# Arcadia-Science/arcadia-microscopy-tools

Measured on AMD Instinct MI355X. Metric: fields-of-view/sec (4x2048^2 uint16) end-to-end segment+props, higher is better.
Workload: dtype f64; 1 GPU; configs[2]: synthetic 4-channel 2048x2048 uint16 FOVs, DAPI Gaussian+Otsu+open/close+EDT+peak markers+watershed nuclei (SEEDED relief, seeds_first: marker pixels spread first in raster order, cannot tie; SURVEY A.8's plain -EDT relief with exact ties is reported under sublines.a8_exact) + clear_border/relabel + morphology and 4-channel intensity regionprops; mode=weak scaling, 192 FOVs per GPU per step, streams_per_gpu=4, fovs_per_launch=48, max_cells_per_fov=2048, distinct_fovs_per_gpu=8, resident_in_hbm=True

## Files before the change

### arcadia_microscopy_tools_amd/csrc/amt_edt.hip

```cpp
#include "amt_internal.h"

constexpr unsigned G_INF = 0xFFFFu;

__global__ void __launch_bounds__(256) edt_zero_words_kernel(const uint8_t* __restrict__ mask, unsigned long long* __restrict__ zw,
                                                             int H, int W, int WW, size_t nwords, int fast) {
    const size_t i = (size_t)blockIdx.x * 256 + threadIdx.x;
    if (i >= nwords) return;
    const int wi = (int)(i % WW);
    const size_t row = i / WW;
    const uint8_t* p = mask + row * W + (size_t)wi * 64;
    const int valid = W - wi * 64 < 64 ? W - wi * 64 : 64;
    unsigned long long z = 0;
    if (fast) {
        uint4 q[4];
#pragma unroll
        for (int j = 0; j < 4; ++j) q[j] = *reinterpret_cast<const uint4*>(p + (16 * j < valid ? 16 * j : 0));
#pragma unroll
        for (int j = 0; j < 4; ++j) {
            const unsigned v[4] = {q[j].x, q[j].y, q[j].z, q[j].w};
            unsigned sixteen = 0;
#pragma unroll
            for (int k = 0; k < 4; ++k) {
                const unsigned nz = ((((v[k] & 0x7F7F7F7Fu) + 0x7F7F7F7Fu) | v[k]) >> 7) & 0x01010101u;
                sixteen |= (((nz ^ 0x01010101u) * 0x01020408u) >> 24) << (4 * k);
            }
            if (16 * j < valid) z |= (unsigned long long)(sixteen & 0xFFFFu) << (16 * j);
        }
    } else {
        for (int k = 0; k < valid; ++k) z |= (unsigned long long)(p[k] == 0) << k;
    }
    zw[i] = z;
}

__device__ __forceinline__ unsigned edt_g_at(const unsigned long long* __restrict__ zr, int WW, int x) {
    const int wi = x >> 6, bit = x & 63;
    const unsigned long long own = zr[wi];
    if ((own >> bit) & 1ull) return 0u;
    unsigned dl = G_INF, dr = G_INF;
    unsigned long long m = own & ((1ull << bit) - 1ull);
    int w = wi;
    while (m == 0 && w > 0) m = zr[--w];
    if (m) dl = (unsigned)(x - (w * 64 + 63 - __clzll((long long)m)));
    m = bit == 63 ? 0ull : (own >> (bit + 1)) << (bit + 1);
    w = wi;
    while (m == 0 && w + 1 < WW) m = zr[++w];
    if (m) dr = (unsigned)(w * 64 + __ffsll((long long)m) - 1 - x);
    const unsigned d = dl < dr ? dl : dr;
    return d >= G_INF ? G_INF : d;
}

template <int EC_ROWS, int EC_HALO>
__global__ void __launch_bounds__(256) edt_bits_kernel(const unsigned long long* __restrict__ zw, int* __restrict__ d2_out,
                                                       double* __restrict__ edt_out, int H, int W, int WW) {
    constexpr int EC_TROWS = EC_ROWS + 2 * EC_HALO;
    __shared__ __attribute__((aligned(16))) unsigned short tile[EC_TROWS][64];
    __shared__ unsigned long long zs[EC_TROWS][3];
    const int lane = threadIdx.x & 63, wave = threadIdx.x >> 6;
    const int wi = blockIdx.x;
    const int y0 = blockIdx.y * EC_ROWS;
    const size_t plane = (size_t)blockIdx.z * H * W;
    const unsigned long long* zp = zw + (size_t)blockIdx.z * H * WW;
    for (int i = threadIdx.x; i < EC_TROWS * 3; i += 256) {
        const int r = i / 3, c = i - r * 3;
        const int y = y0 - EC_HALO + r, w = wi - 1 + c;
        zs[r][c] = (y >= 0 && y < H && w >= 0 && w < WW) ? zp[(size_t)y * WW + w] : 0ull;
    }
    __syncthreads();
    constexpr unsigned BIG = 0x20000u;
    for (int task = threadIdx.x; task < EC_TROWS * 8; task += 256) {
        const int r = task >> 3, b = task & 7;
        const int y = y0 - EC_HALO + r;
        uint4 out = make_uint4(0xFFFFFFFFu, 0xFFFFFFFFu, 0xFFFFFFFFu, 0xFFFFFFFFu);
        if (y >= 0 && y < H) {
            const int bit0 = b * 8, x0 = wi * 64 + bit0;
            const unsigned long long own = zs[r][1];
            const unsigned z8 = (unsigned)(own >> bit0) & 0xffu;
            out = make_uint4(0u, 0u, 0u, 0u);
            if (z8 != 0xffu) {
                unsigned dl = BIG, dr = BIG;
                unsigned long long m = own & ((1ull << bit0) - 1ull);
                int w = wi;
                if (m == 0 && w > 0) {
                    m = zs[r][0];
                    --w;
                    const unsigned long long* zr = zp + (size_t)y * WW;
                    while (m == 0 && w > 0) m = zr[--w];
                }
                if (m) dl = (unsigned)(x0 - (w * 64 + 63 - __clzll((long long)m)));
                const int sh = bit0 + 8;
                m = sh == 64 ? 0ull : (own >> sh) << sh;
                w = wi;
                if (m == 0 && w + 1 < WW) {
                    m = zs[r][2];
                    ++w;
                    const unsigned long long* zr = zp + (size_t)y * WW;
                    while (m == 0 && w + 1 < WW) m = zr[++w];
                }
                if (m) dr = (unsigned)(w * 64 + __ffsll((long long)m) - 1 - (x0 + 7));
                unsigned L[8], R[8];
#pragma unroll
                for (int i = 0; i < 8; ++i) {
                    const unsigned prev = i == 0 ? dl : L[i - 1] + 1u;
                    L[i] = ((z8 >> i) & 1u) ? 0u : (prev < BIG ? prev : BIG);
                }
#pragma unroll
                for (int i = 7; i >= 0; --i) {
                    const unsigned nxt = i == 7 ? dr : R[i + 1] + 1u;
                    R[i] = ((z8 >> i) & 1u) ? 0u : (nxt < BIG ? nxt : BIG);
                }
                unsigned d[8];
#pragma unroll
                for (int i = 0; i < 8; ++i) {
                    const unsigned mn = L[i] < R[i] ? L[i] : R[i];
                    d[i] = mn >= G_INF ? G_INF : mn;
                }
                out.x = d[0] | (d[1] << 16);
                out.y = d[2] | (d[3] << 16);
                out.z = d[4] | (d[5] << 16);
                out.w = d[6] | (d[7] << 16);
            }
        }
        *reinterpret_cast<uint4*>(&tile[r][b * 8]) = out;
    }
    __syncthreads();
    const int c4 = (lane & 15) * 4, rsub = lane >> 4;
    const int xg = wi * 64 + c4;
    if (xg >= W) return;
    const bool vec = xg + 3 < W && (W & 3) == 0 && (!d2_out || (reinterpret_cast<uintptr_t>(d2_out) & 15) == 0) &&
                     (!edt_out || (reinterpret_cast<uintptr_t>(edt_out) & 15) == 0);
#pragma unroll 1
    for (int j = 0; j < EC_ROWS / 16; ++j) {
        const int ly = EC_HALO + wave * (EC_ROWS / 4) + rsub + 4 * j;
        const int y = y0 - EC_HALO + ly;
        if (y >= H) continue;
        unsigned best[4];
        {
            const uint2 gq = *reinterpret_cast<const uint2*>(&tile[ly][c4]);
            const unsigned g0[4] = {gq.x & 0xFFFFu, gq.x >> 16, gq.y & 0xFFFFu, gq.y >> 16};
#pragma unroll
            for (int i = 0; i < 4; ++i) best[i] = g0[i] == G_INF ? 0xFFFFFFFFu : g0[i] * g0[i];
        }
        for (unsigned k = 1; k <= (unsigned)EC_HALO; ++k) {
            const unsigned kk = k * k;
            if (!(kk < best[0] || kk < best[1] || kk < best[2] || kk < best[3])) break;
            const uint2 uq = *reinterpret_cast<const uint2*>(&tile[ly - (int)k][c4]);
            const uint2 dq = *reinterpret_cast<const uint2*>(&tile[ly + (int)k][c4]);
            const unsigned gu[4] = {uq.x & 0xFFFFu, uq.x >> 16, uq.y & 0xFFFFu, uq.y >> 16};
            const unsigned gd[4] = {dq.x & 0xFFFFu, dq.x >> 16, dq.y & 0xFFFFu, dq.y >> 16};
#pragma unroll
            for (int i = 0; i < 4; ++i) {
                const unsigned gm = gu[i] < gd[i] ? gu[i] : gd[i];
                const unsigned c = gm == G_INF ? 0xFFFFFFFFu : kk + gm * gm;
                best[i] = c < best[i] ? c : best[i];
            }
        }
#pragma unroll
        for (int i = 0; i < 4; ++i) {
            unsigned bq = best[i];
            const int x = xg + i;
            if (bq != 0 && x < W) {
                for (unsigned kk = EC_HALO + 1; kk < 65536u && (unsigned long long)kk * kk < bq; ++kk) {
                    const int yu = y - (int)kk, yd = y + (int)kk;
                    if (yu < 0 && yd >= H) break;
                    unsigned gm = G_INF;
                    if (yu >= 0) gm = edt_g_at(zp + (size_t)yu * WW, WW, x);
                    if (yd < H) {
                        const unsigned gd = edt_g_at(zp + (size_t)yd * WW, WW, x);
                        gm = gd < gm ? gd : gm;
                    }
                    if (gm != G_INF) {
                        const unsigned c = kk * kk + gm * gm;
                        bq = c < bq ? c : bq;
                    }
                }
                if (bq > 0x7fffffffu) bq = (unsigned)(y + 1) * (unsigned)(y + 1) + (unsigned)x * (unsigned)x;
            }
            best[i] = bq;
        }
        const size_t i0 = plane + (size_t)y * W + xg;
        if (vec) {
            if (d2_out) *reinterpret_cast<int4*>(d2_out + i0) = make_int4((int)best[0], (int)best[1], (int)best[2], (int)best[3]);
            if (edt_out) {
                *reinterpret_cast<double2*>(edt_out + i0) = make_double2(sqrt((double)best[0]), sqrt((double)best[1]));
                *reinterpret_cast<double2*>(edt_out + i0 + 2) = make_double2(sqrt((double)best[2]), sqrt((double)best[3]));
            }
        } else {
            for (int i = 0; i < 4 && xg + i < W; ++i) {
                if (d2_out) d2_out[i0 + i] = (int)best[i];
                if (edt_out) edt_out[i0 + i] = sqrt((double)best[i]);
            }
        }
    }
}

extern "C" int amt_edt(amt_ctx* ctx, const uint8_t* mask, int32_t* d2_out, double* edt_out, int nplanes, int H,
                       int W) {
    AMT_CHECK_OPERANDS("amt_edt", amt_in("mask", mask, amt_span(1, nplanes, H, W)), amt_out("d2_out", d2_out, amt_span(4, nplanes, H, W)),
                       amt_out("edt_out", edt_out, amt_span(8, nplanes, H, W)));
    AMT_TRY(amt_set_device(ctx));
    AMT_REQUIRE(mask && (d2_out || edt_out) && nplanes >= 0 && H > 0 && W > 0, "edt: bad arguments");
    AMT_REQUIRE(H <= 32768 && W <= 32768, "edt: image larger than 32768 pixels per side");
    if (nplanes == 0) return AMT_OK;
    const size_t tiles64 = (size_t)((W + 63) / 64) * ((H + 63) / 64) * nplanes;
    const int WW = (W + 63) / 64;
    const size_t nwords = (size_t)nplanes * H * WW;
    amt_scratch s(ctx);
    amt_buf<unsigned long long> zw(s, nwords);
    AMT_TRY(s.commit());
    const int fast = W % 16 == 0 && (reinterpret_cast<uintptr_t>(mask) & 15) == 0;
    hipLaunchKernelGGL(edt_zero_words_kernel, dim3((unsigned)((nwords + 255) / 256)), dim3(256), 0, ctx->stream, mask, zw, H,
                       W, WW, nwords, fast);
    AMT_LAUNCH_CHECK();
    if (tiles64 >= 4096 && !edt_out)
        hipLaunchKernelGGL((edt_bits_kernel<64, 16>), dim3(WW, (H + 63) / 64, nplanes), dim3(256), 0, ctx->stream, zw, d2_out,
                           edt_out, H, W, WW);
    else
        hipLaunchKernelGGL((edt_bits_kernel<32, 24>), dim3(WW, (H + 31) / 32, nplanes), dim3(256), 0, ctx->stream, zw, d2_out,
                           edt_out, H, W, WW);
    AMT_LAUNCH_CHECK();
    return AMT_OK;
}

constexpr int PK_MAXM = 16;
constexpr int PKR_ROWS = 64, PKR_IN = 62, PKR_BATCH = 22, PKR_NBATCH = (PKR_ROWS + 2) / PKR_BATCH;
static_assert(PKR_BATCH * PKR_NBATCH == PKR_ROWS + 2, "row batches must tile the strip");
constexpr int PKM_CNT_STRIDE = 32;

template <bool LIST>
__global__ void __launch_bounds__(256) peaks_rows_kernel(const int* __restrict__ d2, const uint8_t* __restrict__ mask,
                                                         uint8_t* __restrict__ peaks, int H, int W, int m,
                                                         int* __restrict__ found, int* __restrict__ fcount, int cap) {
    const int lane = threadIdx.x & 63;
    const int strip = blockIdx.x * 4 + (threadIdx.x >> 6);
    if (strip * PKR_IN >= W) return;
    const size_t base = (size_t)blockIdx.z * H * W;
    const int* D = d2 + base;
    const int x = strip * PKR_IN - 1 + lane;
    const int y0 = blockIdx.y * PKR_ROWS;
    const bool xin = x >= 0 && x < W;
    const bool xok = xin && lane >= 1 && lane <= PKR_IN && x >= m && x < W - m;
    const int side = 2 * m + 1, wsize = side * side;

    const int xc = x < 0 ? 0 : (x < W ? x : W - 1);
    auto load_row = [&](int y) -> int {
        const int yc = y < 0 ? 0 : (y < H ? y : H - 1);
        return D[(size_t)yc * W + xc];
    };
    int npk = 0, mypk = 0;
    auto flush = [&]() {
        int at = 0;
        if (lane == 0) at = atomicAdd(&fcount[(size_t)blockIdx.z * PKM_CNT_STRIDE], npk);
        at = __shfl(at, 0) + lane;
        if (lane < npk && at < cap) found[(size_t)blockIdx.z * cap + at] = mypk;
        npk = 0;
    };
    int cur[PKR_BATCH], nxt[PKR_BATCH];
#pragma unroll
    for (int j = 0; j < PKR_BATCH; ++j) cur[j] = load_row(y0 - 1 + j);
    int v1 = 0, v1l = 0, v1r = 0, h1 = 0, h2 = 0;
    for (int b = 0; b < PKR_NBATCH; ++b) {
        if (b + 1 < PKR_NBATCH) {
#pragma unroll
            for (int j = 0; j < PKR_BATCH; ++j) nxt[j] = load_row(y0 - 1 + (b + 1) * PKR_BATCH + j);
        }
#pragma unroll
        for (int j = 0; j < PKR_BATCH; ++j) {
            const int r = y0 - 1 + b * PKR_BATCH + j;
            const int v0 = (xin && r >= 0 && r < H) ? cur[j] : 0;
            if (__ballot(v0 > 0 || v1 > 0) == 0ull) {
                h2 = h1, h1 = 0, v1 = 0, v1l = 0, v1r = 0;
                continue;
            }
            const int v0l = amt_lane_left(v0), v0r = amt_lane_right(v0);
            int h0 = v0 > v0l ? v0 : v0l;
            h0 = h0 > v0r ? h0 : v0r;
            const int yc = r - 1;
            bool cand = xok && v1 > 0 && yc >= y0 && yc < y0 + PKR_ROWS && yc >= m && yc < H - m;
            if (m >= 1) {
                int nb = h0 > h2 ? h0 : h2;
                nb = nb > v1l ? nb : v1l;
                nb = nb > v1r ? nb : v1r;
                cand = cand && !(nb > v1);
            }
            unsigned long long todo = __ballot(cand);
            while (todo) {
                const int sl = __ffsll((long long)todo) - 1;
                todo &= todo - 1ull;
                const int sv = __shfl(v1, sl);
                const int sx = strip * PKR_IN - 1 + sl;
                bool gt = false;
                for (int k = lane; k < wsize; k += 64) {
                    const int dy = k / side, dx = k - dy * side;
                    gt |= D[(size_t)(yc - m + dy) * W + (sx - m + dx)] > sv;
                }
                const bool hit = __ballot(gt) == 0ull && lane == sl && mask[base + (size_t)yc * W + sx];
                if (hit) peaks[base + (size_t)yc * W + sx] = 1;
                if (LIST && __ballot(hit) != 0ull) {
                    if (lane == npk) mypk = yc * W + sx;
                    if (++npk == 64) flush();
                }
            }
            h2 = h1, h1 = h0;
            v1 = v0, v1l = v0l, v1r = v0r;
        }
#pragma unroll
        for (int j = 0; j < PKR_BATCH; ++j) cur[j] = nxt[j];
    }
    if (LIST && npk) flush();
}

__global__ void __launch_bounds__(256) peaks_unwrite_kernel(const int* __restrict__ list, const int* __restrict__ count,
                                                            const int* __restrict__ status, uint8_t* __restrict__ peaks,
                                                            size_t n, int cap) {
    uint8_t* o = peaks + (size_t)blockIdx.y * n;
    if (status[blockIdx.y] < 0) {
        for (size_t i = (size_t)blockIdx.x * 256 + threadIdx.x; i < n; i += (size_t)gridDim.x * 256) o[i] = 0;
        return;
    }
    const int K = count[blockIdx.y] < cap ? count[blockIdx.y] : cap;
    const int* lst = list + (size_t)blockIdx.y * cap;
    for (int k = blockIdx.x * 256 + threadIdx.x; k < K; k += gridDim.x * 256) o[lst[k]] = 0;
}

extern "C" int amt_peak_mask(amt_ctx* ctx, const int32_t* d2, const uint8_t* mask, uint8_t* peaks, int nplanes, int H,
                             int W, int min_distance, const int32_t* prev_list, const int32_t* prev_count, int capacity,
                             const int32_t* prev_status) {
    AMT_REQUIRE(!prev_list == !prev_count && !prev_list == !prev_status,
                "peak_mask: the previous run's peak lists, counts and label counts go together");
    AMT_REQUIRE(!prev_list || capacity >= 1, "peak_mask: the previous run's list capacity must be positive");
    AMT_CHECK_OPERANDS("amt_peak_mask", amt_in("d2", d2, amt_span(4, nplanes, H, W)), amt_in("mask", mask, amt_span(1, nplanes, H, W)),
                       amt_out("peaks", peaks, amt_span(1, nplanes, H, W)),
                       amt_in("prev_list", prev_list, amt_span(4, nplanes, capacity)),
                       amt_in("prev_count", prev_count, amt_span(4, nplanes)),
                       amt_in("prev_status", prev_status, amt_span(4, nplanes)));
    AMT_TRY(amt_set_device(ctx));
    AMT_REQUIRE(d2 && mask && peaks && nplanes >= 0 && H > 0 && W > 0, "peak_mask: bad arguments");
    AMT_REQUIRE(min_distance >= 0 && min_distance <= PK_MAXM, "peak_mask: min_distance %d out of range 0..%d",
                min_distance, PK_MAXM);
    if (nplanes == 0) return AMT_OK;
    const int m = min_distance;
    if (prev_list) {
        hipLaunchKernelGGL(peaks_unwrite_kernel, dim3(amt_grid_for((size_t)capacity, 256, 64), nplanes), dim3(256), 0,
                           ctx->stream, prev_list, prev_count, prev_status, peaks, (size_t)H * W, capacity);
        AMT_LAUNCH_CHECK();
    } else {
        AMT_HIP_CHECK(hipMemsetAsync(peaks, 0, (size_t)nplanes * H * W, ctx->stream));
    }
    const int nstrips = (W + PKR_IN - 1) / PKR_IN;
    dim3 grid((nstrips + 3) / 4, (H + PKR_ROWS - 1) / PKR_ROWS, nplanes);
    hipLaunchKernelGGL(peaks_rows_kernel<false>, grid, dim3(256), 0, ctx->stream, d2, mask, peaks, H, W, m, (int*)nullptr,
                       (int*)nullptr, 0);
    AMT_LAUNCH_CHECK();
    return AMT_OK;
}

constexpr int PKM_TIER = AMT_PEAK_MARKERS_LDS_TIER;
constexpr int PKM_THREADS = 1024;
static_assert(2 * PKM_TIER * sizeof(int) <= 36 * 1024 - 256, "list + parents of the LDS tier stay below 36 KB");

__global__ void __launch_bounds__(256) peaks_clear_kernel(const int* __restrict__ list, const int* __restrict__ count,
                                                          const int* __restrict__ status, uint8_t* __restrict__ peaks,
                                                          int* __restrict__ markers, int* __restrict__ fcount, size_t n,
                                                          int cap) {
    if (blockIdx.x == 0 && threadIdx.x == 0) fcount[(size_t)blockIdx.y * PKM_CNT_STRIDE] = 0;
    uint8_t* pk = peaks + (size_t)blockIdx.y * n;
    int* mk = markers + (size_t)blockIdx.y * n;
    if (status[blockIdx.y] < 0) {
        for (size_t i = (size_t)blockIdx.x * 256 + threadIdx.x; i < n; i += (size_t)gridDim.x * 256) pk[i] = 0, mk[i] = 0;
        return;
    }
    const int K = count[blockIdx.y] < cap ? count[blockIdx.y] : cap;
    const int* lst = list + (size_t)blockIdx.y * cap;
    for (int k = blockIdx.x * 256 + threadIdx.x; k < K; k += gridDim.x * 256) {
        const int p = lst[k];
        pk[p] = 0;
        mk[p] = 0;
    }
}

__device__ __forceinline__ void pkm_exchange(int* a, int i, int l, int n) {
    if (l < n) {
        const int u = a[i], v = a[l];
        if (u > v) a[i] = v, a[l] = u;
    }
}
__device__ __forceinline__ void pkm_sort(int* a, int n) {
    int n2 = 1;
    while (n2 < n) n2 <<= 1;
    const int pairs = n2 >> 1;
    for (int k = 2; k <= n2; k <<= 1) {
        const int hk = k >> 1;
        for (int t = threadIdx.x; t < pairs; t += PKM_THREADS) {
            const int i = ((t & ~(hk - 1)) << 1) | (t & (hk - 1));
            pkm_exchange(a, i, i ^ (k - 1), n);
        }
        __syncthreads();
        for (int j = hk >> 1; j > 0; j >>= 1) {
            for (int t = threadIdx.x; t < pairs; t += PKM_THREADS) {
                const int i = ((t & ~(j - 1)) << 1) | (t & (j - 1));
                pkm_exchange(a, i, i | j, n);
            }
            __syncthreads();
        }
    }
}

template <bool LDS>
__device__ __forceinline__ int pkm_label(int* lst, int* par, int K, int W, int conn8, int* __restrict__ mk,
                                         int* __restrict__ kl, int* wsum) {
    const int tid = threadIdx.x;
    pkm_sort(lst, K);
    for (int k = tid; k < K; k += PKM_THREADS) {
        par[k] = k;
        if (kl) kl[k] = lst[k];
    }
    __syncthreads();
    for (int k = tid; k < K; k += PKM_THREADS) {
        const int p = lst[k];
        const int y = p / W, x = p - y * W;
        if (x > 0 && k > 0 && lst[k - 1] == p - 1) {
            if (LDS) lds_union(par, k, k - 1); else uf_union(par, k, k - 1);
        }
        if (y == 0) continue;
        const int north = p - W;
        int lo = 0, hi = k;
        while (lo < hi) {
            const int mid = (lo + hi) >> 1;
            if (lst[mid] < north) lo = mid + 1; else hi = mid;
        }
        const bool up = lst[lo] == north;
        if (up) {
            if (LDS) lds_union(par, k, lo); else uf_union(par, k, lo);
        }
        if (conn8) {
// ... 20 lines not shown
    int rank = incl - mine, total = 0;
    for (int w = 0; w < PKM_THREADS / 64; ++w) {
        if (w < wave) rank += wsum[w];
        total += wsum[w];
    }
    for (int k = b; k < e; ++k)
        if (par[k] == k) par[k] = ~(rank++);
    __syncthreads();
    for (int k = tid; k < K; k += PKM_THREADS) {
        int v = par[k];
        if (v >= 0) v = par[v];
        mk[lst[k]] = -v;
    }
    return total;
}

__global__ void __launch_bounds__(PKM_THREADS) sp_markers_kernel(int* found, const int* __restrict__ fcount, int* gpar,
                                                                 int* __restrict__ markers, int* __restrict__ count_dev,
                                                                 int* __restrict__ keep_list, int* __restrict__ keep_count,
                                                                 size_t n, int W, int cap, int conn8) {
    __shared__ int s_lst[PKM_TIER], s_par[PKM_TIER];
    __shared__ int s_wsum[PKM_THREADS / 64];
    const int plane = blockIdx.x;
    const int K = fcount[(size_t)plane * PKM_CNT_STRIDE];
    if (K > cap) {
        if (threadIdx.x == 0) {
            count_dev[plane] = -1;
            if (keep_count) keep_count[plane] = 0;
        }
        return;
    }
    int* fl = found + (size_t)plane * cap;
    int* mk = markers + (size_t)plane * n;
    int* kl = keep_list ? keep_list + (size_t)plane * cap : nullptr;
    int nroots;
    if (K <= PKM_TIER) {
        for (int k = threadIdx.x; k < K; k += PKM_THREADS) s_lst[k] = fl[k];
        __syncthreads();
        nroots = pkm_label<true>(s_lst, s_par, K, W, conn8, mk, kl, s_wsum);
    } else {
        nroots = pkm_label<false>(fl, gpar + (size_t)plane * cap, K, W, conn8, mk, kl, s_wsum);
    }
    if (threadIdx.x == 0) {
        count_dev[plane] = nroots;
        if (keep_count) keep_count[plane] = K;
    }
}

extern "C" int amt_peak_markers(amt_ctx* ctx, const int32_t* d2, const uint8_t* mask, uint8_t* peaks, int32_t* markers,
                                int32_t* count_dev, int nplanes, int H, int W, int min_distance, int connectivity,
                                int capacity, int32_t* keep_list, int32_t* keep_count) {
    AMT_REQUIRE(!keep_list == !keep_count, "peak_markers: keep_list and keep_count go together");
    AMT_CHECK_OPERANDS("amt_peak_markers", amt_in("d2", d2, amt_span(4, nplanes, H, W)), amt_in("mask", mask, amt_span(1, nplanes, H, W)),
                       amt_out("peaks", peaks, amt_span(1, nplanes, H, W)), amt_out("markers", markers, amt_span(4, nplanes, H, W)),
                       amt_out("count_dev", count_dev, amt_span(4, nplanes)),
                       amt_out("keep_list", keep_list, amt_span(4, nplanes, capacity)),
                       amt_out("keep_count", keep_count, amt_span(4, nplanes)));
    AMT_REQUIRE(d2 && mask && peaks && markers && count_dev && nplanes >= 0 && H > 0 && W > 0,
                "peak_markers: bad arguments");
    AMT_REQUIRE(min_distance >= 0 && min_distance <= PK_MAXM, "peak_markers: min_distance %d out of range 0..%d",
                min_distance, PK_MAXM);
    AMT_REQUIRE(connectivity == 1 || connectivity == 2, "peak_markers: connectivity must be 1 or 2");
    AMT_REQUIRE(capacity >= 1, "peak_markers: capacity must be positive");
    AMT_REQUIRE((size_t)H * W < 0x7fffffffull, "peak_markers: plane too large");
    AMT_TRY(amt_set_device(ctx));
    if (nplanes == 0) return AMT_OK;
    const size_t n = (size_t)H * W;
    const size_t capn = (size_t)nplanes * capacity;
    amt_scratch s(ctx);
    amt_buf<int> found(s, capn);
    amt_buf<int> parent(s, capn);
    amt_buf<int> fcount(s, (size_t)nplanes * PKM_CNT_STRIDE);
    AMT_TRY(s.commit());
    if (keep_list) {
        hipLaunchKernelGGL(peaks_clear_kernel, dim3(amt_grid_for((size_t)capacity, 256, 64), nplanes), dim3(256), 0,
                           ctx->stream, (const int*)keep_list, (const int*)keep_count, (const int*)count_dev, peaks, markers,
                           (int*)fcount, n, capacity);
        AMT_LAUNCH_CHECK();
    } else {
        AMT_HIP_CHECK(hipMemsetAsync(peaks, 0, (size_t)nplanes * n, ctx->stream));
        AMT_HIP_CHECK(hipMemsetAsync(markers, 0, (size_t)nplanes * n * sizeof(int32_t), ctx->stream));
        AMT_HIP_CHECK(hipMemsetAsync(fcount, 0, (size_t)nplanes * PKM_CNT_STRIDE * sizeof(int), ctx->stream));
    }
    const int nstrips = (W + PKR_IN - 1) / PKR_IN;
    dim3 grid((nstrips + 3) / 4, (H + PKR_ROWS - 1) / PKR_ROWS, nplanes);
    hipLaunchKernelGGL(peaks_rows_kernel<true>, grid, dim3(256), 0, ctx->stream, d2, mask, peaks, H, W, min_distance,
                       (int*)found, (int*)fcount, capacity);
    AMT_LAUNCH_CHECK();
    hipLaunchKernelGGL(sp_markers_kernel, dim3(nplanes), dim3(PKM_THREADS), 0, ctx->stream, (int*)found,
                       (const int*)fcount, (int*)parent, markers, count_dev, keep_list, keep_count, n, W, capacity,
                       connectivity == 2 ? 1 : 0);
    AMT_LAUNCH_CHECK();
    return AMT_OK;
}
```

### arcadia_microscopy_tools_amd/csrc/amt_props.hip

```cpp
#include "amt_internal.h"
#include "amt_perlabel.h"

#include <vector>

typedef unsigned long long u64;

enum { A_N = 0, A_SY, A_SX, A_SYY, A_SXX, A_SXY, A_C1, A_C2, A_C3, A_NACC };

__global__ void __launch_bounds__(256) rp_init_kernel(u64* __restrict__ acc, int* __restrict__ bbox, size_t nlab) {
    for (size_t i = (size_t)blockIdx.x * 256 + threadIdx.x; i < nlab; i += (size_t)gridDim.x * 256) {
        if (acc)
            for (int k = 0; k < A_NACC; ++k) acc[i * A_NACC + k] = 0;
        bbox[i * 4 + 0] = 0x7fffffff;
        bbox[i * 4 + 1] = 0x7fffffff;
        bbox[i * 4 + 2] = -1;
        bbox[i * 4 + 3] = -1;
    }
}

__device__ __forceinline__ double diff_of_products(u64 a, u64 b, u64 c, u64 d) {
    u64 lo1 = a * b, hi1 = __umul64hi(a, b);
    u64 lo2 = c * d, hi2 = __umul64hi(c, d);
    bool neg = (hi1 < hi2) || (hi1 == hi2 && lo1 < lo2);
    u64 hi, lo;
// ... 469 lines not shown
    const int2* r = rows + (size_t)plane * cap + off;
    int2* CL = chainL + (size_t)plane * 3 * cap + 3 * off;
    int2* CR = chainR + (size_t)plane * 3 * cap + 3 * off;
    int nl = 0, nr = 0;
    for (int Y = 2 * miny - 1; Y <= 2 * maxy + 1; ++Y) {
        int mn = 0x7fffffff, mx = -0x7fffffff;
        if (Y & 1) {
            int ya = (Y - 1) / 2, yb = (Y + 1) / 2;
            if (Y < 0) {
                ya = -1;
                yb = 0;
            }
            if (ya >= miny && ya <= maxy) {
                int2 e = r[ya - miny];
                if (e.y >= e.x) {
                    mn = min(mn, 2 * e.x);
                    mx = max(mx, 2 * e.y);
                }
            }
            if (yb >= miny && yb <= maxy) {
                int2 e = r[yb - miny];
                if (e.y >= e.x) {
                    mn = min(mn, 2 * e.x);
                    mx = max(mx, 2 * e.y);
                }
            }
        } else {
            int2 e = r[Y / 2 - miny];
            if (e.y >= e.x) {
                mn = 2 * e.x - 1;
                mx = 2 * e.y + 1;
            }
        }
        if (mx < mn) continue;
        while (nl >= 2) {
            int2 p0 = CL[nl - 2], p1 = CL[nl - 1];
            long long cr = (long long)(p1.x - p0.x) * (mn - p0.y) - (long long)(p1.y - p0.y) * (Y - p0.x);
            if (cr <= 0) --nl; else break;
        }
        CL[nl++] = make_int2(Y, mn);
        while (nr >= 2) {
            int2 p0 = CR[nr - 2], p1 = CR[nr - 1];
            long long cr = (long long)(p1.x - p0.x) * (mx - p0.y) - (long long)(p1.y - p0.y) * (Y - p0.x);
            if (cr >= 0) --nr; else break;
        }
        CR[nr++] = make_int2(Y, mx);
    }
    long long count = 0;
    int il = 0, ir = 0;
    for (int y = miny; y <= maxy; ++y) {
        const int Y = 2 * y;
        while (il + 1 < nl && CL[il + 1].x <= Y) ++il;
        while (ir + 1 < nr && CR[ir + 1].x <= Y) ++ir;
        long long xmin, xmax;
        {
            int2 p0 = CL[il];
            if (p0.x == Y || il + 1 >= nl) {
                xmin = ceil_div(p0.y, 2);
            } else {
                int2 p1 = CL[il + 1];
                long long dY = p1.x - p0.x;
                long long num = (long long)p0.y * dY + (long long)(p1.y - p0.y) * (Y - p0.x);
                xmin = ceil_div(num, 2 * dY);
            }
        }
        {
            int2 p0 = CR[ir];
            if (p0.x == Y || ir + 1 >= nr) {
                xmax = floor_div(p0.y, 2);
            } else {
                int2 p1 = CR[ir + 1];
                long long dY = p1.x - p0.x;
                long long num = (long long)p0.y * dY + (long long)(p1.y - p0.y) * (Y - p0.x);
                xmax = floor_div(num, 2 * dY);
            }
        }
        if (CROWS) crows[(size_t)plane * cap + off + (y - miny)] = make_int2((int)xmin, (int)xmax);
        else if (xmax >= xmin) count += xmax - xmin + 1;
    }
    if (!CROWS) rp_write_convex(trow, (double)count);
}

constexpr int HULL_CH = 2 * HULL_HMAX + 1;
__device__ __forceinline__ int floor_div32(int a, int b) {
    const int q = a / b;
    return (a % b != 0 && a < 0) ? q - 1 : q;
}
__device__ __forceinline__ int ceil_div32(int a, int b) {
    const int q = a / b;
    return (a % b != 0 && a > 0) ? q + 1 : q;
}
template <bool CROWS>
__global__ void __launch_bounds__(64) rp_hull_lds_kernel(const int* __restrict__ bbox, const int* __restrict__ hoff,
                                                         const int* __restrict__ htot, const int2* __restrict__ rows,
                                                         size_t cap, double* __restrict__ table, int max_label,
                                                         int2* __restrict__ crows) {
    __shared__ unsigned short s_rows[HULL_HMAX * 32];
    __shared__ unsigned short s_ch[HULL_CH * 64];
    const int plane = blockIdx.y;
    const int lane = threadIdx.x, side = lane & 1, pr = lane >> 1;
    const int l = blockIdx.x * 32 + pr;
    if (l >= max_label) return;
    const size_t li = (size_t)plane * max_label + l;
    double* trow = CROWS ? nullptr : table + li * AMT_RP_NCOLS;
    const int miny = bbox[li * 4 + 0], x0 = bbox[li * 4 + 1], maxy = bbox[li * 4 + 2], x1 = bbox[li * 4 + 3];
    if (maxy < miny) {
        if (!CROWS && side == 0) trow[AMT_RP_AREA_CONVEX] = 0.0;
        return;
    }
    const int h = maxy - miny + 1;
    if (h > HULL_HMAX || x1 - x0 + 1 > HULL_WMAX) return;
    const size_t off = (size_t)hoff[li];
    if ((size_t)htot[plane] > cap || off + (size_t)h > cap) {
        if (!CROWS && side == 0) rp_write_convex(trow, __longlong_as_double(0x7ff8000000000000ll));
        return;
    }
    const int2* r = rows + (size_t)plane * cap + off;
    for (int k0 = side; k0 < h; k0 += 16) {
        int2 e[8];
#pragma unroll
        for (int u = 0; u < 8; ++u) e[u] = r[min(k0 + 2 * u, h - 1)];
#pragma unroll
        for (int u = 0; u < 8; ++u)
            if (k0 + 2 * u < h)
                s_rows[(k0 + 2 * u) * 32 + pr] =
                    e[u].y >= e[u].x ? (unsigned short)((e[u].x - x0) | ((e[u].y - x0) << 8)) : (unsigned short)255;
    }
    __builtin_amdgcn_s_waitcnt(0);
    __builtin_amdgcn_wave_barrier();
    int nc = 0;
    for (int Yr = 0; Yr <= 2 * h; ++Yr) {
        int mn = 0x7fffffff, mx = -1;
        if (!(Yr & 1)) {
            const int ka = (Yr >> 1) - 1, kb = Yr >> 1;
            if (ka >= 0) {
                const unsigned e = s_rows[ka * 32 + pr];
                if ((e >> 8) >= (e & 255)) {
                    mn = min(mn, 2 * (int)(e & 255) + 1);
                    mx = max(mx, 2 * (int)(e >> 8) + 1);
                }
            }
            if (kb < h) {
                const unsigned e = s_rows[kb * 32 + pr];
                if ((e >> 8) >= (e & 255)) {
                    mn = min(mn, 2 * (int)(e & 255) + 1);
                    mx = max(mx, 2 * (int)(e >> 8) + 1);
                }
            }
        } else {
            const unsigned e = s_rows[(Yr >> 1) * 32 + pr];
            if ((e >> 8) >= (e & 255)) {
                mn = 2 * (int)(e & 255);
                mx = 2 * (int)(e >> 8) + 2;
            }
        }
        if (mx < mn) continue;
        const int val = side ? mx : mn;
        while (nc >= 2) {
            const int v0 = s_ch[(nc - 2) * 64 + lane], v1 = s_ch[(nc - 1) * 64 + lane];
            const int cr = ((v1 >> 9) - (v0 >> 9)) * (val - (v0 & 511)) - ((v1 & 511) - (v0 & 511)) * (Yr - (v0 >> 9));
            if (side ? cr >= 0 : cr <= 0) --nc; else break;
        }
        s_ch[(nc++) * 64 + lane] = (unsigned short)((Yr << 9) | val);
    }
    int count = 0;
    int ic = 0;
    for (int k = 0; k < h; ++k) {
        const int Yr = 2 * k + 1;
        while (ic + 1 < nc && (int)(s_ch[(ic + 1) * 64 + lane] >> 9) <= Yr) ++ic;
        int b;
        const int v0 = s_ch[ic * 64 + lane];
        if ((v0 >> 9) == Yr || ic + 1 >= nc) {
            b = side ? floor_div32((v0 & 511) - 1, 2) : ceil_div32((v0 & 511) - 1, 2);
        } else {
            const int v1 = s_ch[(ic + 1) * 64 + lane];
            const int dY = (v1 >> 9) - (v0 >> 9);
            const int num = ((v0 & 511) - 1) * dY + ((v1 & 511) - (v0 & 511)) * (Yr - (v0 >> 9));
            b = side ? floor_div32(num, 2 * dY) : ceil_div32(num, 2 * dY);
        }
        const int other = __shfl_xor(b, 1);
        const int xmin = side ? other : b, xmax = side ? b : other;
        if (CROWS) {
            if (side == 0) crows[(size_t)plane * cap + off + k] = make_int2(xmin + x0, xmax + x0);
        } else if (xmax >= xmin) {
            count += xmax - xmin + 1;
        }
    }
    if (!CROWS && side == 0) rp_write_convex(trow, (double)count);
}

__global__ void __launch_bounds__(256) rp_final_kernel(const u64* __restrict__ acc, const int* __restrict__ bbox,
                                                       double* __restrict__ table, size_t nlab) {
    for (size_t i = (size_t)blockIdx.x * 256 + threadIdx.x; i < nlab; i += (size_t)gridDim.x * 256) {
        const u64* A = acc + i * A_NACC;
        const int* B = bbox + i * 4;
        double* t = table + i * AMT_RP_NCOLS;
        const u64 n = A[A_N];
        if (n == 0) {
            for (int k = 0; k < AMT_RP_NCOLS; ++k)
                if (k != AMT_RP_AREA_CONVEX) t[k] = 0.0;
            continue;
        }
        const double dn = (double)n;
        t[AMT_RP_AREA] = dn;
        t[AMT_RP_CENTROID_Y] = (double)A[A_SY] / dn;
        t[AMT_RP_CENTROID_X] = (double)A[A_SX] / dn;
        t[AMT_RP_BBOX_Y0] = (double)B[0];
        t[AMT_RP_BBOX_X0] = (double)B[1];
        t[AMT_RP_BBOX_Y1] = (double)(B[2] + 1);
        t[AMT_RP_BBOX_X1] = (double)(B[3] + 1);
        const double SQ2 = 1.4142135623730951;
        t[AMT_RP_PERIMETER] = (double)A[A_C1] + (double)A[A_C2] * SQ2 + (double)A[A_C3] * ((1.0 + SQ2) / 2.0);
        const double Nyy = diff_of_products(n, A[A_SYY], A[A_SY], A[A_SY]);
        const double Nxx = diff_of_products(n, A[A_SXX], A[A_SX], A[A_SX]);
        const double Nxy = diff_of_products(n, A[A_SXY], A[A_SX], A[A_SY]);
        const double n2 = dn * dn;
        const double a = Nxx / n2;
        const double c = Nyy / n2;
        const double b = -Nxy / n2;
        const double tr = (a + c) * 0.5;
        const double hd = (a - c) * 0.5;
        const double rad = sqrt(hd * hd + b * b);
        double l1 = tr + rad, l2 = tr - rad;
        l1 = l1 < 0.0 ? 0.0 : l1;
        l2 = l2 < 0.0 ? 0.0 : l2;
        t[AMT_RP_AXIS_MAJOR] = 4.0 * sqrt(l1);
        t[AMT_RP_AXIS_MINOR] = 4.0 * sqrt(l2);
        t[AMT_RP_ECCENTRICITY] = l1 == 0.0 ? 0.0 : sqrt(1.0 - l2 / l1);
        double orient;
        if (Nxx == Nyy) {
            orient = (Nxy > 0.0) ? -0.78539816339744828 : 0.78539816339744828;
        } else {
            orient = 0.5 * atan2(-2.0 * b, c - a);
        }
        t[AMT_RP_ORIENTATION] = orient;
    }
}

extern "C" int amt_regionprops(amt_ctx* ctx, const int32_t* labels, const uint16_t* intensity, int C, double* table_dev,
                               double* itable_dev, int nplanes, int H, int W, int max_label) {
    AMT_REQUIRE(labels && (table_dev || itable_dev) && nplanes >= 0 && H > 0 && W > 0 && max_label >= 0,
                "regionprops: bad arguments");
    AMT_REQUIRE(!intensity == !itable_dev && (!itable_dev || C >= 1),
                "regionprops: the intensity planes (C >= 1) and the intensity table go together");
    AMT_CHECK_OPERANDS("amt_regionprops", amt_in("labels", labels, amt_span(4, nplanes, H, W)),
                       amt_in("intensity", intensity, amt_span(2, nplanes, C, H, W)),
                       amt_out("table_dev", table_dev, amt_span(8, nplanes, max_label, AMT_RP_NCOLS)),
                       amt_out("itable_dev", itable_dev, amt_span(8, nplanes, max_label, C, 4)));
    AMT_TRY(amt_set_device(ctx));
    const bool want_morph = table_dev != nullptr;
    if (nplanes == 0 || max_label == 0) return AMT_OK;
    const size_t n = (size_t)H * W;
    const size_t nlab = (size_t)nplanes * max_label;
    const size_t cap = want_morph ? n : 1;
    amt_scratch s(ctx);
    amt_buf<u64> acc(s, nlab * A_NACC);
    amt_buf<int> bbox(s, nlab * 4);
    amt_buf<int> hoff(s, nlab);
    amt_buf<int> htot(s, nplanes);
    amt_buf<int2> rows(s, (size_t)nplanes * cap);
    amt_buf<int2> chainL(s, (size_t)nplanes * 3 * cap);
    amt_buf<int2> chainR(s, (size_t)nplanes * 3 * cap);
// ... 880 lines not shown
```

Baseline: 16720 FOV/s.

## Add vectorized 4-pixel-per-lane peak detection kernel with software-pipelined row batches

```diff
diff --git a/arcadia_microscopy_tools_amd/csrc/amt_edt.hip b/arcadia_microscopy_tools_amd/csrc/amt_edt.hip
--- a/arcadia_microscopy_tools_amd/csrc/amt_edt.hip
+++ b/arcadia_microscopy_tools_amd/csrc/amt_edt.hip
@@ -309,6 +309,163 @@
     if (LIST && npk) flush();
 }
 
+constexpr int PKS_ROWS = 64, PKS_COLS = 256, PKS_BATCH = 6, PKS_NBATCH = (PKS_ROWS + 2) / PKS_BATCH;
+static_assert(PKS_BATCH * PKS_NBATCH == PKS_ROWS + 2, "row batches must tile the strip");
+
+template <bool LIST>
+__global__ void __launch_bounds__(256) peaks_rows4_kernel(const int* __restrict__ d2, const uint8_t* __restrict__ mask,
+                                                          uint8_t* __restrict__ peaks, int H, int W, int m,
+                                                          int* __restrict__ found, int* __restrict__ fcount, int cap) {
+    const int lane = threadIdx.x & 63;
+    const int x0 = (blockIdx.x * 4 + (threadIdx.x >> 6)) * PKS_COLS;
+    if (x0 >= W) return;
+    const size_t base = (size_t)blockIdx.z * H * W;
+    const int* D = d2 + base;
+    const uint8_t* M = mask + base;
+    const int y0 = blockIdx.y * PKS_ROWS;
+    const int xg = x0 + 4 * lane;
+    const bool gin = xg < W;
+    const int xgc = gin ? xg : W - 4;
+    const int xh = lane == 0 ? x0 - 1 : x0 + PKS_COLS;
+    const bool hin = (lane == 0 || lane == 63) && xh >= 0 && xh < W;
+    const int xhc = hin ? xh : 0;
+    const unsigned hsel = lane == 0 ? 0x000000ffu : (lane == 63 ? 0xff000000u : 0u);
+    unsigned xsel = 0;
+#pragma unroll
+    for (int i = 0; i < 4; ++i) xsel |= (xg + i >= m && xg + i < W - m) ? 0xffu << (8 * i) : 0u;
+    const int side = 2 * m + 1, wsize = side * side;
+
+    auto load_mask = [&](int t) -> unsigned {
+        const int r = y0 - 1 + t;
+        const int rc = r < H ? r : H - 1;
+        return *reinterpret_cast<const unsigned*>(M + (size_t)rc * W + xgc);
+    };
+    int npk = 0, mypk = 0;
+    auto flush = [&]() {
+        int at = 0;
+        if (lane == 0) at = atomicAdd(&fcount[(size_t)blockIdx.z * PKM_CNT_STRIDE], npk);
+        at = __shfl(at, 0) + lane;
+        if (lane < npk && at < cap) found[(size_t)blockIdx.z * cap + at] = mypk;
+        npk = 0;
+    };
+    unsigned mp = 0, mc = 0, hdp = 0, hdc = 0;
+    auto issue = [&](int b, const unsigned (&mk)[PKS_BATCH], int4 (&dn)[PKS_BATCH], int (&hn)[PKS_BATCH],
+                     unsigned (&ma)[PKS_BATCH]) {
+#pragma unroll
+        for (int j = 0; j < PKS_BATCH; ++j) {
+            const int tn = b * PKS_BATCH + j + 1;
+            const unsigned mn = (gin && tn <= PKS_ROWS && y0 - 1 + tn < H) ? mk[j] : 0u;
+            const unsigned hdn = mn | ((unsigned)amt_lane_left((int)mn) >> 24) | ((unsigned)amt_lane_right((int)mn) & 0xffu);
+            const int r = y0 - 1 + b * PKS_BATCH + j;
+            const bool rin = r >= 0 && r < H;
+            int4 v = make_int4(0, 0, 0, 0);
+            if (((hdp | hdc | hdn) != 0u) && rin && gin) v = *reinterpret_cast<const int4*>(D + (size_t)r * W + xg);
+            int hv = 0;
+            if ((((mp | mc | mn) & hsel) != 0u) && rin && hin) hv = D[(size_t)r * W + xhc];
+            dn[j] = v, hn[j] = hv, ma[j] = mc;
+            hdp = hdc, hdc = hdn, mp = mc, mc = mn;
+        }
+    };
+    int e1[6] = {0, 0, 0, 0, 0, 0}, e2[6] = {0, 0, 0, 0, 0, 0};
+    unsigned m1 = 0;
+    auto process = [&](int b, const int4 (&dc)[PKS_BATCH], const int (&hc)[PKS_BATCH], const unsigned (&ma)[PKS_BATCH]) {
+#pragma unroll
+        for (int j = 0; j < PKS_BATCH; ++j) {
+            const int4 v0 = dc[j];
+            const int vl = amt_lane_left(v0.w), vr = amt_lane_right(v0.x);
+            const int e0[6] = {lane == 0 ? hc[j] : vl, v0.x, v0.y, v0.z, v0.w, lane == 63 ? hc[j] : vr};
+            const int yc = y0 - 2 + b * PKS_BATCH + j;
+            const unsigned cm = m1 & xsel;
+            if (yc >= m && yc < H - m && __ballot(cm != 0u) != 0ull) {
+                unsigned cb = 0;
+#pragma unroll
+                for (int i = 0; i < 4; ++i) {
+                    const int c = e1[i + 1];
+                    bool cand = ((cm >> (8 * i)) & 0xffu) != 0u && c > 0;
+                    if (m >= 1) {
+                        int nb = e0[i] > e0[i + 1] ? e0[i] : e0[i + 1];
+                        nb = nb > e0[i + 2] ? nb : e0[i + 2];
+                        nb = nb > e2[i] ? nb : e2[i];
+                        nb = nb > e2[i + 1] ? nb : e2[i + 1];
+                        nb = nb > e2[i + 2] ? nb : e2[i + 2];
+                        nb = nb > e1[i] ? nb : e1[i];
+                        nb = nb > e1[i + 2] ? nb : e1[i + 2];
+                        cand = cand && !(nb > c);
+                    }
+                    cb |= cand ? 1u << i : 0u;
+                }
+                unsigned long long todo = __ballot(cb != 0u);
+                while (todo) {
+                    const int sl = __ffsll((long long)todo) - 1;
+                    const unsigned scb = (unsigned)__shfl((int)cb, sl);
+                    const int i = __ffs((int)scb) - 1;
+                    if ((scb & (scb - 1u)) == 0u) todo &= todo - 1ull;
+                    if (lane == sl) cb &= cb - 1u;
+                    const int sv = __shfl(i == 0 ? e1[1] : (i == 1 ? e1[2] : (i == 2 ? e1[3] : e1[4])), sl);
+                    const int sx = x0 + 4 * sl + i;
+                    bool gt = false;
+                    for (int k = lane; k < wsize; k += 64) {
+                        const int dy = k / side, dx = k - dy * side;
+                        gt |= D[(size_t)(yc - m + dy) * W + (sx - m + dx)] > sv;
+                    }
+                    if (__ballot(gt) == 0ull) {
+                        if (lane == sl) peaks[base + (size_t)yc * W + sx] = 1;
+                        if (LIST) {
+                            if (lane == npk) mypk = yc * W + sx;
+                            if (++npk == 64) flush();
+                        }
+                    }
+                }
+            }
+#pragma unroll
+            for (int i = 0; i < 6; ++i) e2[i] = e1[i], e1[i] = e0[i];
+            m1 = ma[j];
+        }
+    };
+
+    unsigned mka[PKS_BATCH], mkb[PKS_BATCH], maa[PKS_BATCH], mab[PKS_BATCH];
+    int4 da[PKS_BATCH], db[PKS_BATCH];
+    int ha[PKS_BATCH], hb[PKS_BATCH];
+#pragma unroll
+    for (int j = 0; j < PKS_BATCH; ++j) mka[j] = load_mask(1 + j);
+#pragma unroll
+    for (int j = 0; j < PKS_BATCH; ++j) mkb[j] = load_mask(PKS_BATCH + 1 + j);
+    issue(0, mka, da, ha, maa);
+#pragma unroll 1
+    for (int b = 0; b < PKS_NBATCH; b += 2) {
+        if (b + 2 < PKS_NBATCH) {
+#pragma unroll
+            for (int j = 0; j < PKS_BATCH; ++j) mka[j] = load_mask((b + 2) * PKS_BATCH + 1 + j);
+        }
+        if (b + 1 < PKS_NBATCH) issue(b + 1, mkb, db, hb, mab);
+        process(b, da, ha, maa);
+        if (b + 1 >= PKS_NBATCH) break;
+        if (b + 3 < PKS_NBATCH) {
+#pragma unroll
+            for (int j = 0; j < PKS_BATCH; ++j) mkb[j] = load_mask((b + 3) * PKS_BATCH + 1 + j);
+        }
+        if (b + 2 < PKS_NBATCH) issue(b + 2, mka, da, ha, maa);
+        process(b + 1, db, hb, mab);
+    }
+    if (LIST && npk) flush();
+}
+
+template <bool LIST>
+static void peaks_rows_launch(amt_ctx* ctx, const int32_t* d2, const uint8_t* mask, uint8_t* peaks, int nplanes, int H, int W,
+                              int m, int* found, int* fcount, int cap) {
+    if (W % 4 == 0 && (reinterpret_cast<uintptr_t>(d2) & 15) == 0 && (reinterpret_cast<uintptr_t>(mask) & 3) == 0) {
+        const int nstrips = (W + PKS_COLS - 1) / PKS_COLS;
+        dim3 grid((nstrips + 3) / 4, (H + PKS_ROWS - 1) / PKS_ROWS, nplanes);
+        hipLaunchKernelGGL(peaks_rows4_kernel<LIST>, grid, dim3(256), 0, ctx->stream, d2, mask, peaks, H, W, m, found, fcount,
+                           cap);
+    } else {
+        const int nstrips = (W + PKR_IN - 1) / PKR_IN;
+        dim3 grid((nstrips + 3) / 4, (H + PKR_ROWS - 1) / PKR_ROWS, nplanes);
+        hipLaunchKernelGGL(peaks_rows_kernel<LIST>, grid, dim3(256), 0, ctx->stream, d2, mask, peaks, H, W, m, found, fcount,
+                           cap);
+    }
+}
+
 __global__ void __launch_bounds__(256) peaks_unwrite_kernel(const int* __restrict__ list, const int* __restrict__ count,
                                                             const int* __restrict__ status, uint8_t* __restrict__ peaks,
                                                             size_t n, int cap) {
@@ -346,10 +503,7 @@
     } else {
         AMT_HIP_CHECK(hipMemsetAsync(peaks, 0, (size_t)nplanes * H * W, ctx->stream));
     }
-    const int nstrips = (W + PKR_IN - 1) / PKR_IN;
-    dim3 grid((nstrips + 3) / 4, (H + PKR_ROWS - 1) / PKR_ROWS, nplanes);
-    hipLaunchKernelGGL(peaks_rows_kernel<false>, grid, dim3(256), 0, ctx->stream, d2, mask, peaks, H, W, m, (int*)nullptr,
-                       (int*)nullptr, 0);
+    peaks_rows_launch<false>(ctx, d2, mask, peaks, nplanes, H, W, m, nullptr, nullptr, 0);
     AMT_LAUNCH_CHECK();
     return AMT_OK;
 }
@@ -536,10 +690,7 @@
         AMT_HIP_CHECK(hipMemsetAsync(markers, 0, (size_t)nplanes * n * sizeof(int32_t), ctx->stream));
         AMT_HIP_CHECK(hipMemsetAsync(fcount, 0, (size_t)nplanes * PKM_CNT_STRIDE * sizeof(int), ctx->stream));
     }
-    const int nstrips = (W + PKR_IN - 1) / PKR_IN;
-    dim3 grid((nstrips + 3) / 4, (H + PKR_ROWS - 1) / PKR_ROWS, nplanes);
-    hipLaunchKernelGGL(peaks_rows_kernel<true>, grid, dim3(256), 0, ctx->stream, d2, mask, peaks, H, W, min_distance,
-                       (int*)found, (int*)fcount, capacity);
+    peaks_rows_launch<true>(ctx, d2, mask, peaks, nplanes, H, W, min_distance, (int*)found, (int*)fcount, capacity);
     AMT_LAUNCH_CHECK();
     hipLaunchKernelGGL(sp_markers_kernel, dim3(nplanes), dim3(PKM_THREADS), 0, ctx->stream, (int*)found,
                        (const int*)fcount, (int*)parent, markers, count_dev, keep_list, keep_count, n, W, capacity,
```

After: 16520 FOV/s. -1.2%, worse.

## Use 16x16 EDT column regions and a register-cached convex-hull stack

Applied to the files above, without the earlier changes.

```diff
diff --git a/arcadia_microscopy_tools_amd/csrc/amt_edt.hip b/arcadia_microscopy_tools_amd/csrc/amt_edt.hip
--- a/arcadia_microscopy_tools_amd/csrc/amt_edt.hip
+++ b/arcadia_microscopy_tools_amd/csrc/amt_edt.hip
@@ -49,11 +49,16 @@
     return d >= G_INF ? G_INF : d;
 }
 
-template <int EC_ROWS, int EC_HALO>
+template <int EC_ROWS, int EC_HALO, int EC_RR>
 __global__ void __launch_bounds__(256) edt_bits_kernel(const unsigned long long* __restrict__ zw, int* __restrict__ d2_out,
                                                        double* __restrict__ edt_out, int H, int W, int WW) {
     constexpr int EC_TROWS = EC_ROWS + 2 * EC_HALO;
-    __shared__ __attribute__((aligned(16))) unsigned short tile[EC_TROWS][64];
+    constexpr int EC_RC = 256 / EC_RR, EC_LPR = EC_RC / 4, EC_NCG = 64 / EC_RC;
+    constexpr int EC_TS = EC_RR == 4 ? 64 : EC_RR == 8 ? 96 : 80;
+    static_assert(EC_RR == 4 || EC_RR == 8 || EC_RR == 16, "regions of 4 x 64, 8 x 32 or 16 x 16 pixels");
+    static_assert(EC_ROWS % EC_RR == 0 && EC_ROWS % 16 == 0, "the tile is a whole number of regions per wave");
+    static_assert((EC_TS * 2) % 16 == 0, "16-byte stores into the rows of the tile");
+    __shared__ __attribute__((aligned(16))) unsigned short tile[EC_TROWS][EC_TS];
     __shared__ unsigned long long zs[EC_TROWS][3];
     const int lane = threadIdx.x & 63, wave = threadIdx.x >> 6;
     const int wi = blockIdx.x;
@@ -123,16 +128,18 @@
         *reinterpret_cast<uint4*>(&tile[r][b * 8]) = out;
     }
     __syncthreads();
-    const int c4 = (lane & 15) * 4, rsub = lane >> 4;
-    const int xg = wi * 64 + c4;
-    if (xg >= W) return;
-    const bool vec = xg + 3 < W && (W & 3) == 0 && (!d2_out || (reinterpret_cast<uintptr_t>(d2_out) & 15) == 0) &&
-                     (!edt_out || (reinterpret_cast<uintptr_t>(edt_out) & 15) == 0);
+    const int rsub = lane / EC_LPR;
+    const bool aligned = (W & 3) == 0 && (!d2_out || (reinterpret_cast<uintptr_t>(d2_out) & 15) == 0) &&
+                         (!edt_out || (reinterpret_cast<uintptr_t>(edt_out) & 15) == 0);
 #pragma unroll 1
     for (int j = 0; j < EC_ROWS / 16; ++j) {
-        const int ly = EC_HALO + wave * (EC_ROWS / 4) + rsub + 4 * j;
+        const int q = wave * (EC_ROWS / 16) + j;
+        const int c4 = (q % EC_NCG) * EC_RC + (lane % EC_LPR) * 4;
+        const int ly = EC_HALO + (q / EC_NCG) * EC_RR + rsub;
+        const int xg = wi * 64 + c4;
         const int y = y0 - EC_HALO + ly;
-        if (y >= H) continue;
+        if (y >= H || xg >= W) continue;
+        const bool vec = aligned && xg + 3 < W;
         unsigned best[4];
         {
             const uint2 gq = *reinterpret_cast<const uint2*>(&tile[ly][c4]);
@@ -212,11 +219,11 @@
                        W, WW, nwords, fast);
     AMT_LAUNCH_CHECK();
     if (tiles64 >= 4096 && !edt_out)
-        hipLaunchKernelGGL((edt_bits_kernel<64, 16>), dim3(WW, (H + 63) / 64, nplanes), dim3(256), 0, ctx->stream, zw, d2_out,
-                           edt_out, H, W, WW);
+        hipLaunchKernelGGL((edt_bits_kernel<64, 16, 16>), dim3(WW, (H + 63) / 64, nplanes), dim3(256), 0, ctx->stream, zw,
+                           d2_out, edt_out, H, W, WW);
     else
-        hipLaunchKernelGGL((edt_bits_kernel<32, 24>), dim3(WW, (H + 31) / 32, nplanes), dim3(256), 0, ctx->stream, zw, d2_out,
-                           edt_out, H, W, WW);
+        hipLaunchKernelGGL((edt_bits_kernel<32, 24, 16>), dim3(WW, (H + 31) / 32, nplanes), dim3(256), 0, ctx->stream, zw,
+                           d2_out, edt_out, H, W, WW);
     AMT_LAUNCH_CHECK();
     return AMT_OK;
 }
diff --git a/arcadia_microscopy_tools_amd/csrc/amt_props.hip b/arcadia_microscopy_tools_amd/csrc/amt_props.hip
--- a/arcadia_microscopy_tools_amd/csrc/amt_props.hip
+++ b/arcadia_microscopy_tools_amd/csrc/amt_props.hip
@@ -575,14 +575,43 @@
 }
 
 constexpr int HULL_CH = 2 * HULL_HMAX + 1;
-__device__ __forceinline__ int floor_div32(int a, int b) {
-    const int q = a / b;
-    return (a % b != 0 && a < 0) ? q - 1 : q;
-}
-__device__ __forceinline__ int ceil_div32(int a, int b) {
-    const int q = a / b;
-    return (a % b != 0 && a > 0) ? q + 1 : q;
-}
+static_assert(2 * HULL_HMAX < (1 << 7) && 2 * HULL_WMAX + 1 < (1 << 9), "a chain vertex is (Yr << 9 | Xr) in 16 bits");
+static_assert(HULL_WMAX <= 255, "a row is (min | max << 8) in 16 bits, 255 | 0 << 8 the empty one");
+static_assert(2 * (2 * HULL_WMAX + 1) * (2 * HULL_HMAX) < (1 << 20) && 2 * (2 * HULL_HMAX) < (1 << 9),
+              "hull_floor_div: |num| < 2^20, d < 2^9");
+__device__ __forceinline__ int hull_floor_div(int num, int d, int* rem) {
+    int q = __float2int_rd((float)num * __builtin_amdgcn_rcpf((float)d));
+    int r = num - q * d;
+    if (r < 0) {
+        --q;
+        r += d;
+    } else if (r >= d) {
+        ++q;
+        r -= d;
+    }
+    *rem = r;
+    return q;
+}
+struct hull_stack {
+    unsigned short* ch;
+    int nc, t0, t1, t2;
+    __device__ __forceinline__ void push(int Yr, int val, int side) {
+        while (nc >= 2) {
+            const int cr = ((t1 >> 9) - (t0 >> 9)) * (val - (t0 & 511)) - ((t1 & 511) - (t0 & 511)) * (Yr - (t0 >> 9));
+            if (!(side ? cr >= 0 : cr <= 0)) break;
+            --nc;
+            t1 = t0;
+            t0 = t2;
+            if (nc >= 3) t2 = ch[(nc - 3) * 64];
+        }
+        const int v = (Yr << 9) | val;
+        ch[nc * 64] = (unsigned short)v;
+        t2 = t0;
+        t0 = t1;
+        t1 = v;
+        ++nc;
+    }
+};
 template <bool CROWS>
 __global__ void __launch_bounds__(64) rp_hull_lds_kernel(const int* __restrict__ bbox, const int* __restrict__ hoff,
                                                          const int* __restrict__ htot, const int2* __restrict__ rows,
@@ -621,56 +650,36 @@
     }
     __builtin_amdgcn_s_waitcnt(0);
     __builtin_amdgcn_wave_barrier();
-    int nc = 0;
-    for (int Yr = 0; Yr <= 2 * h; ++Yr) {
-        int mn = 0x7fffffff, mx = -1;
-        if (!(Yr & 1)) {
-            const int ka = (Yr >> 1) - 1, kb = Yr >> 1;
-            if (ka >= 0) {
-                const unsigned e = s_rows[ka * 32 + pr];
-                if ((e >> 8) >= (e & 255)) {
-                    mn = min(mn, 2 * (int)(e & 255) + 1);
-                    mx = max(mx, 2 * (int)(e >> 8) + 1);
-                }
-            }
-            if (kb < h) {
-                const unsigned e = s_rows[kb * 32 + pr];
-                if ((e >> 8) >= (e & 255)) {
-                    mn = min(mn, 2 * (int)(e & 255) + 1);
-                    mx = max(mx, 2 * (int)(e >> 8) + 1);
-                }
-            }
-        } else {
-            const unsigned e = s_rows[(Yr >> 1) * 32 + pr];
-            if ((e >> 8) >= (e & 255)) {
-                mn = 2 * (int)(e & 255);
-                mx = 2 * (int)(e >> 8) + 2;
-            }
-        }
-        if (mx < mn) continue;
-        const int val = side ? mx : mn;
-        while (nc >= 2) {
-            const int v0 = s_ch[(nc - 2) * 64 + lane], v1 = s_ch[(nc - 1) * 64 + lane];
-            const int cr = ((v1 >> 9) - (v0 >> 9)) * (val - (v0 & 511)) - ((v1 & 511) - (v0 & 511)) * (Yr - (v0 >> 9));
-            if (side ? cr >= 0 : cr <= 0) --nc; else break;
-        }
-        s_ch[(nc++) * 64 + lane] = (unsigned short)((Yr << 9) | val);
-    }
+    hull_stack st{s_ch + lane, 0, 0, 0, 0};
+    unsigned prev = 255u;
+    for (int k = 0; k <= h; ++k) {
+        const unsigned cur = k < h ? (unsigned)s_rows[k * 32 + pr] : 255u;
+        const bool pe = (prev >> 8) >= (prev & 255u), ce = (cur >> 8) >= (cur & 255u);
+        if (pe || ce) {
+            const int mn = min(pe ? (int)(prev & 255u) : 0x7fff, ce ? (int)(cur & 255u) : 0x7fff);
+            const int mx = max(pe ? (int)(prev >> 8) : -1, ce ? (int)(cur >> 8) : -1);
+            st.push(2 * k, 2 * (side ? mx : mn) + 1, side);
+        }
+        if (ce) st.push(2 * k + 1, side ? 2 * (int)(cur >> 8) + 2 : 2 * (int)(cur & 255u), side);
+        prev = cur;
+    }
+    const int nc = st.nc;
     int count = 0;
     int ic = 0;
+    int v0 = s_ch[lane], v1 = nc > 1 ? (int)s_ch[64 + lane] : v0;
     for (int k = 0; k < h; ++k) {
         const int Yr = 2 * k + 1;
-        while (ic + 1 < nc && (int)(s_ch[(ic + 1) * 64 + lane] >> 9) <= Yr) ++ic;
-        int b;
-        const int v0 = s_ch[ic * 64 + lane];
-        if ((v0 >> 9) == Yr || ic + 1 >= nc) {
-            b = side ? floor_div32((v0 & 511) - 1, 2) : ceil_div32((v0 & 511) - 1, 2);
-        } else {
-            const int v1 = s_ch[(ic + 1) * 64 + lane];
-            const int dY = (v1 >> 9) - (v0 >> 9);
-            const int num = ((v0 & 511) - 1) * dY + ((v1 & 511) - (v0 & 511)) * (Yr - (v0 >> 9));
-            b = side ? floor_div32(num, 2 * dY) : ceil_div32(num, 2 * dY);
-        }
+        while (ic + 1 < nc && (v1 >> 9) <= Yr) {
+            ++ic;
+            v0 = v1;
+            if (ic + 1 < nc) v1 = s_ch[(ic + 1) * 64 + lane];
+        }
+        const bool last = ic + 1 >= nc;
+        const int dY = last ? 1 : (v1 >> 9) - (v0 >> 9);
+        const int num = ((v0 & 511) - 1) * dY + (last ? 0 : ((v1 & 511) - (v0 & 511)) * (Yr - (v0 >> 9)));
+        int rem;
+        const int q = hull_floor_div(num, 2 * dY, &rem);
+        const int b = side ? q : q + (rem != 0);
         const int other = __shfl_xor(b, 1);
         const int xmin = side ? other : b, xmax = side ? b : other;
         if (CROWS) {
```

Measured after the change: 16690 FOV/s before, 16950 FOV/s after (median of 6 runs). +1.6%, better.
